# waldstein94/Stratified-Transformer

Measured on AMD Instinct MI355X. Metric: points/sec through StratifiedAttention fwd+bwd, 100k-pt scene, higher is better.
Workload: dtype f32

## Files before the change

include/pointops2_hip.h:

```cpp
#ifndef POINTOPS2_HIP_H
#define POINTOPS2_HIP_H

#include <stddef.h>
#include <stdint.h>

#ifdef __cplusplus
extern "C" {
#endif

void pointops2_set_stream(void *hip_stream);
void *pointops2_get_stream(void);
const char *pointops2_last_error(void);
int pointops2_abi_version(void);
void pointops2_diag_set_fps_patience(unsigned long long ticks_100mhz);


void furthestsampling_cuda_launcher(int b, int n, const float *xyz, const int *offset,
                                    const int *new_offset, float *tmp, int *idx);

void knnquery_cuda_launcher(int m, int nsample, const float *xyz, const float *new_xyz,
                            const int *offset, const int *new_offset, int *idx, float *dist2);

void grouping_forward_cuda_launcher(int m, int nsample, int c, const float *input, const int *idx, float *output);
void grouping_backward_cuda_launcher(int m, int nsample, int c, const float *grad_output, const int *idx, float *grad_input);
// ... 103 lines not shown
void segment_softmax_forward_launcher(int N, int M, int h, const float *src, const int *offsets, float *out);
void segment_softmax_backward_launcher(int N, int M, int h, const float *out, const float *grad_out,
                                       const int *offsets, float *grad_src);
void pointops2_bbox_launcher(int N, const float *xyz, float *out6);
size_t pointops2_index_workspace_bytes(int N);
void pointops2_window_partition_launcher(int N, int b, const float *xyz, const int *offset, const float *bbox6, float size,
                                         float shift, int key_bits, int *cluster, int *order, int *starts, int *n_windows,
                                         void *ws, size_t ws_bytes);
size_t pointops2_row_order_workspace_bytes(int N);
void pointops2_row_order_launcher(int N, int M, const int *offsets, const int *index1, int *order, void *ws, size_t ws_bytes);
size_t pointops2_partitions4_workspace_bytes(int N);
void pointops2_window_partitions4_launcher(int N, int b, const float *xyz, const int *offset, const float *bbox6, float window,
                                           int *cluster, int *order, int *starts, int *n_windows, int *overflow, void *ws,
                                           size_t ws_bytes);
void pointops2_window_coord_launcher(int N, const float *xyz, const float *bbox6, float window, int shifted, float *wc);
void pointops2_sampled_buckets_launcher(int N, int m, const int *sample_idx, const int *l_order, const int *l_starts,
                                        const int *l_n_windows, int *sampled, int *ls, int *ls_starts, void *ws, size_t ws_bytes);
void pointops2_pairs_count_launcher(int N, const int *s_cluster, const int *s_starts, const int *l_cluster, const int *ls,
                                    const int *ls_starts, const float *wc, int *offsets, void *ws, size_t ws_bytes);
void pointops2_pairs_fill_launcher(int N, const float *xyz, float window, float quant, const int *s_cluster, const int *s_order,
                                   const int *s_starts, const int *l_cluster, const int *ls, const int *ls_starts, const float *wc,
                                   const int *offsets, int *index_0, int *index_1, int *rel_idx);

void csr_expand_launcher(int N, int M, const int *offsets, int *index0);

void pointops2_csr_matches_launcher(int N, int M, const int *offsets, const void *index, int index_is_int64, int *bad);

void window_logits_softmax_forward_launcher(int N, int M, int h, int hdim, const float *q, const int *index_q_offsets,
                                             const float *k, const int *index_k, const float *table_q,
                                             const float *table_k, const int *rel_idx, float *attn);
// ... 215 lines not shown
```

stratified_transformer_amd/_lib.py:

```python
import ctypes
import os
import subprocess

import torch

_HERE = os.path.dirname(os.path.abspath(__file__))
LIB_PATH = os.path.join(_HERE, "lib", "libpointops2_hip.so")
CSRC = os.path.join(_HERE, "csrc")
_lib = None

I, U, P, Z, F, D = ctypes.c_int, ctypes.c_uint, ctypes.c_void_p, ctypes.c_size_t, ctypes.c_float, ctypes.c_double
Q = ctypes.c_longlong


class LaunchOpts(ctypes.Structure):
    _fields_ = [("table_rows", I), ("key_rows", I), ("csc_offsets", P), ("csc_pair", P), ("csc_query", P), ("row_order", P),
                ("row_order_rows", I), ("workspace", P), ("workspace_bytes", Z), ("point_count", I), ("batch_count", I),
                ("fps_prev_idx", P), ("fps_prev_new_offset", P), ("fps_unordered", I)]


def with_table_rows(opts, L):
    opts = opts if opts is not None else LaunchOpts()
    opts.table_rows = int(L)
    return opts
# ... 31 lines not shown
    "subtraction_forward_cuda_launcher": [I, I, I, P, P, P, P],
    "subtraction_backward_cuda_launcher": [I, I, I, P, P, P, P],
    "aggregation_forward_cuda_launcher": [I, I, I, I, P, P, P, P, P],
    "aggregation_backward_cuda_launcher": [I, I, I, I, P, P, P, P, P, P, P, P],
    "segment_softmax_forward_launcher": [I, I, I, P, P, P],
    "window_logits_softmax_forward_launcher": [I, I, I, I, P, P, P, P, P, P, P, P],
    "window_attention_backward_launcher": [I, I, I, I] + [P] * 18,
    "segment_softmax_backward_launcher": [I, I, I, P, P, P, P],
    "csr_expand_launcher": [I, I, P, P],
    "pointops2_csr_matches_launcher": [I, I, P, P, I, P],
    "pointops2_bbox_launcher": [I, P, P],
    "pointops2_window_partition_launcher": [I, I, P, P, P, F, F, I, P, P, P, P, P, Z],
    "pointops2_window_partitions4_launcher": [I, I, P, P, P, F, P, P, P, P, P, P, Z],
    "pointops2_row_order_launcher": [I, I, P, P, P, P, Z],
    "pointops2_window_coord_launcher": [I, P, P, F, I, P],
    "pointops2_sampled_buckets_launcher": [I, I, P, P, P, P, P, P, P, P, Z],
    "pointops2_pairs_count_launcher": [I, P, P, P, P, P, P, P, P, Z],
    "pointops2_pairs_fill_launcher": [I, P, F, F, P, P, P, P, P, P, P, P, P, P, P],
    "pointops2_voxel_keys_launcher": [I, I, P, ctypes.c_double, P],
    "pointops2_crop_dist_launcher": [I, I, P, I, P],
    "pointops2_cell_plan_count_launcher": [I, I, P, P, P, P, P, P, P, P, P, P, P, P, P, P, Z],
    "pointops2_cell_plan_prepare_launcher": [I, I, P, P, P, P, P, P, Z],
    "pointops2_cell_plan_sizes_launcher": [I, P, P, P, P, P, P, P, P, P, P, P, P, P, Z],
    "pointops2_cell_plan_fill_launcher": [I, P, F, F, I, P, P, P, P, P, P, P, P, P, P, P, P],
    "pointops2_swin_quant_launcher": [I, P, P, F, F, I, P],
    "pointops2_swin_pairs_rel_launcher": [I, I, P, P, P, I, P],
    "pointops2_swin_cell_fill_launcher": [I, I, I] + [P] * 13,
    "cell_attention_forward_launcher": [P, I, I, I] + [P] * 9,
    "cell_attention_backward_launcher": [P, I, I, I] + [P] * 16,
    "cell_attention_forward_bf16_launcher": [P, I, I, I] + [P] * 9,
# ... 33 lines not shown
    "pointops2_augment_pass_launcher": [I] * 6 + [P] * 10,
    "pointops2_augment_blur_launcher": [Q, I, I, P, P, P],
    "optim_adamw_step_launcher": [I, I, P, P, Z, P, P, I],
    "optim_step_launcher": [I, I, I, P, P, Z, P, P, I, D, P],
}
RESULTS = {
    "pointops2_get_stream": ([], P),
    "pointops2_last_error": ([], ctypes.c_char_p),
    "pointops2_abi_version": ([], I),
    "pointops2_csc_workspace_bytes": ([I, I], Z),
    "pointops2_fps_workspace_bytes": ([I, I], Z),
    "pointops2_knn_workspace_bytes": ([I, I, I], Z),
    "pointops2_index_workspace_bytes": ([I], Z),
    "pointops2_partitions4_workspace_bytes": ([I], Z),
    "pointops2_row_order_workspace_bytes": ([I], Z),
    "pointops2_cell_plan_workspace_bytes": ([I], Z),
    "pointops2_cell_forward_variant": ([P, I, I, I, I], I),
    "pointops2_evaltile_max_parts": ([], I),
    "pointops2_optim_workspace_bytes": ([I, I], Z),
    "pointops2_optim_step_workspace_bytes": ([I, I, Q], Z),
}
OPTIM_KINDS = {"adamw": 0, "sgd": 1}

CELL_FWD = {"error": -1, "none": 0, "mfma64": 1, "mfma80": 2, "valu80": 3, "valu160": 4}
ROW_TYPES = {torch.float32: 0, torch.float16: 1, torch.bfloat16: 2}
ACTIVATIONS = {"none": 0, "relu": 1, "leaky_relu": 2, "tanh": 3}


def cell_forward_variant(plan, h, L, bf16=False, hdim=16):
    arg = None if plan is None else plan.c_arg() if hasattr(plan, "c_arg") else ctypes.byref(plan)
# ... 72 lines not shown
```

stratified_transformer_amd/csrc/fps_bucket.hip:

```cpp
#include "fps_common.h"
#include <hipcub/hipcub.hpp>
#include <cstdlib>

namespace p2 {

constexpr int FPS_MAX_BUCKETS = 2048;

__device__ __forceinline__ unsigned row0_max_u32(unsigned v) {
    v = dpp_step<0xB1, 0xF>(v);
    v = dpp_step<0x4E, 0xF>(v);
    v = dpp_step<0x141, 0xF>(v);
    v = dpp_step<0x140, 0xF>(v);
    return (unsigned)__builtin_amdgcn_readfirstlane((int)v);
}
__device__ __forceinline__ unsigned long long wmax64(unsigned long long v) {
    const unsigned hi = (unsigned)(v >> 32), lo = (unsigned)v;
    const unsigned mh = wave_max_u32(hi);
    const unsigned ml = wave_max_u32(hi == mh ? lo : 0u);
    return ((unsigned long long)mh << 32) | ml;
}

constexpr int BBOX_T = 1024;
__global__ __launch_bounds__(BBOX_T) void fps_bbox_kernel(const float *__restrict__ xyz, const int *__restrict__ offset,
                                                          float *__restrict__ bbox) {
// ... 569 lines not shown
        hipLaunchKernelGGL((fps_bucket_kernel<NBL, FPS_NW, true>), dim3(b), dim3(FPS_NW * 64), 0, st, Bref, log2B, BSZ, xyz, offset, new_offset, pts,
                           rank, prev_idx, prev_offset, verified, idx);
    else
        hipLaunchKernelGGL((fps_bucket_kernel<NBL, FPS_NW, false>), dim3(b), dim3(FPS_NW * 64), 0, st, Bref, log2B, BSZ, xyz, offset, new_offset, pts,
                           rank, prev_idx, prev_offset, verified, idx);
}

static size_t al(size_t x) { return (x + 255) & ~(size_t)255; }
static int bits_for(int b) {
    int r = 1;
    while ((1 << r) < b) r++;
    return r;
}
constexpr int FPS_HEAD = 256;

static size_t fps_cub_bytes(int b, int N) {
    size_t bytes = 0;
    (void)hipcub::DeviceRadixSort::SortPairs(nullptr, bytes, (const unsigned long long *)nullptr, (unsigned long long *)nullptr,
                                             (const int *)nullptr, (int *)nullptr, N, 0, 32 + bits_for(b), (hipStream_t) nullptr);
    return bytes;
}

__global__ void fps_head_offsets_kernel(int b, int head, const int *__restrict__ new_offset, int *__restrict__ head_offset) {
    if (threadIdx.x != 0 || blockIdx.x != 0) return;
    int acc = 0;
    for (int i = 0; i < b; i++) {
        const int m = new_offset[i] - (i ? new_offset[i - 1] : 0);
        acc += min(m, head);
        head_offset[i] = acc;
    }
}

bool fps_bucket_launch(const Launch &ln, int b, int n, int Bref, int log2B, const float *xyz, const int *offset,
                       const int *new_offset, int *idx) {
    const pointops2_launch_opts &o = ln.opts;
    const int N_total = o.point_count;
// ... 9 lines not shown
    int *vals_in = (int *)p; p += f4;
    unsigned long long *keys_in = (unsigned long long *)p; p += f8;
    unsigned long long *keys_out = (unsigned long long *)p; p += f8;
    float *bbox = (float *)p; p += al((size_t)b * 6 * 4);
    int *inv = (int *)p; p += f4;
    unsigned long long *thr = (unsigned long long *)p; p += f8;
    int *first_bad = (int *)p; p += al((size_t)b * 4);
    void *xchg = p; p += al((size_t)b * LZ_XCHG);
    int *head_offset = (int *)p; p += al((size_t)b * 4);
    int *head_idx = (int *)p; p += al((size_t)b * FPS_HEAD * 4);
    void *cub_tmp = p;
    size_t cub_bytes = o.workspace_bytes - (size_t)(p - reinterpret_cast<char *>(o.workspace));
    if (o.fps_prev_idx == nullptr) {
        hipLaunchKernelGGL(fps_bbox_kernel, dim3(b), dim3(BBOX_T), 0, st, xyz, offset, bbox);
        hipLaunchKernelGGL(fps_morton_kernel, dim3(div_up(N_total, 256)), dim3(256), 0, st, N_total, b, xyz, offset, bbox, keys_in, vals_in);
        hipError_t e = hipcub::DeviceRadixSort::SortPairs(cub_tmp, cub_bytes, keys_in, keys_out, (const int *)vals_in, sorig, N_total, 0,
                                                          32 + bits_for(b), st);
        if (e != hipSuccess) { set_error(hipGetErrorString(e)); return true; }
        hipLaunchKernelGGL(fps_gather_kernel, dim3(div_up(N_total, 256)), dim3(256), 0, st, N_total, b, Bref, log2B, xyz, offset, sorig, pts, rank, inv);
    }
    const int *verified = nullptr;
    if (!o.fps_unordered) {
        hipLaunchKernelGGL(fps_verify_init_kernel, dim3(div_up(b, 64)), dim3(64), 0, st, b, offset, new_offset, first_bad);
        hipLaunchKernelGGL(fps_verify_threshold_kernel, dim3(1, b), dim3(VER_T), 0, st, Bref, log2B, 1, xyz, offset, new_offset, first_bad, thr);
        hipLaunchKernelGGL(fps_verify_scan_kernel, dim3(div_up(n, VER_P), b), dim3(VER_T), 0, st, Bref, log2B, 1, 64, xyz, offset, new_offset, thr, first_bad);
        hipLaunchKernelGGL(fps_verify_threshold_kernel, dim3(div_up(n, VER_P), b), dim3(VER_T), 0, st, Bref, log2B, 64, xyz, offset, new_offset, first_bad, thr);
        hipLaunchKernelGGL(fps_verify_scan_kernel, dim3(div_up(n, VER_P), b), dim3(VER_T), 0, st, Bref, log2B, 64, 0x7fffffff, xyz, offset, new_offset, thr, first_bad);
        hipLaunchKernelGGL(fps_rebuild_kernel, dim3(div_up(n, VER_P), b), dim3(VER_T), 0, st, xyz, offset, o.fps_prev_new_offset, first_bad, inv, pts);
        verified = first_bad;
    }
    const int BSZ = 64 * div_up(n, 64 * FPS_MAX_BUCKETS);
    const int nbuckets = div_up(n, BSZ);
// ... 37 lines not shown
```

stratified_transformer_amd/csrc/index.hip:

```cpp
#include "common.h"
#include <hipcub/hipcub.hpp>

namespace p2 {

__device__ __forceinline__ float div_floor(float a, float b) {
    if (b == 0.f) return __fdiv_rn(a, b);
    const float mod = fmodf(a, b);
    float div = __fdiv_rn(__fsub_rn(a, mod), b);
    if ((mod != 0.f) && ((b < 0.f) != (mod < 0.f))) div = __fsub_rn(div, 1.f);
    float floordiv;
    if (div != 0.f) {
        floordiv = floorf(div);
        if (__fsub_rn(div, floordiv) > 0.5f) floordiv = __fadd_rn(floordiv, 1.f);
    } else {
        floordiv = copysignf(0.f, __fdiv_rn(a, b));
    }
    return floordiv;
}

__global__ __launch_bounds__(1024) void bbox_kernel(int N, const float *__restrict__ xyz, float *__restrict__ out6) {
    __shared__ float red[6][16];
    const int tid = threadIdx.x;
    float mn[3] = {INFINITY, INFINITY, INFINITY}, mx[3] = {-INFINITY, -INFINITY, -INFINITY};
    for (int i0 = tid; i0 < N; i0 += 4 * 1024) {
// ... 352 lines not shown
        unsigned w = (jl >= nd && !coord_differs(wc, i, j)) ? 0x80000000u : 0u;
#pragma unroll
        for (int a = 0; a < 3; a++) {
            const int b = min(max(qi[a] - q[(size_t)j * 3 + a] + bias, 0), L - 1);
            w |= (unsigned)b << (8 * a);
        }
        row[jl] = w;
        if (il == 0) {
            cell_keys[kb + jl] = j;
            kcell[kb + jl] = cid;
        }
    }
}

static size_t al(size_t x) { return (x + 255) & ~(size_t)255; }
static size_t sort64_bytes(int N) {
    size_t bytes = 0;
    (void)hipcub::DeviceRadixSort::SortPairs(nullptr, bytes, (const unsigned long long *)nullptr, (unsigned long long *)nullptr,
                                             (const int *)nullptr, (int *)nullptr, N, 0, 64, (hipStream_t) nullptr);
    return bytes;
}
static size_t sort32_bytes(int N) {
    size_t bytes = 0;
    (void)hipcub::DeviceRadixSort::SortPairs(nullptr, bytes, (const unsigned *)nullptr, (unsigned *)nullptr, (const int *)nullptr, (int *)nullptr, N, 0, 32,
                                             (hipStream_t) nullptr);
    return bytes;
}
__global__ void row_order_key_kernel(int N, int M, const int *__restrict__ offs, const int *__restrict__ idx1, unsigned *__restrict__ keys,
                                     int *__restrict__ vals) {
    const int i = blockIdx.x * blockDim.x + threadIdx.x;
    if (i >= N) return;
    const int s = offs[i], e = offs[i + 1];
    keys[i] = (s >= 0 && s < e && s < M) ? (unsigned)idx1[s] : 0xffffffffu;
    vals[i] = i;
}
static size_t scan_bytes(int N) {
    size_t bytes = 0;
    (void)hipcub::DeviceScan::InclusiveSum(nullptr, bytes, (const int *)nullptr, (int *)nullptr, N, (hipStream_t) nullptr);
    size_t b2 = 0;
    (void)hipcub::DeviceScan::ExclusiveSum(nullptr, b2, (const int *)nullptr, (int *)nullptr, N, (hipStream_t) nullptr);
    return bytes > b2 ? bytes : b2;
}
// ... 21 lines not shown
                                         size_t ws_bytes) {
    const hipStream_t st = begin_launch().stream;
    if (N <= 0) return;
    if (ws_bytes < pointops2_index_workspace_bytes(N)) { set_error("pointops2_window_partition: workspace too small"); return; }
    char *p = reinterpret_cast<char *>(ws);
    unsigned long long *keys_in = (unsigned long long *)p; p += al((size_t)N * 8);
    unsigned long long *keys_out = (unsigned long long *)p; p += al((size_t)N * 8);
    int *vals_in = (int *)p; p += al(((size_t)N + 1) * 4);
    int *flags = (int *)p; p += al(((size_t)N + 1) * 4);
    int *rank = (int *)p; p += al(((size_t)N + 1) * 4);
    p += al(((size_t)N + 1) * 4);
    void *tmp = p;
    size_t tmp_bytes = ws_bytes - (size_t)(p - reinterpret_cast<char *>(ws));
    const int g = div_up(N, 256);
    hipLaunchKernelGGL(voxel_key_kernel, dim3(g), dim3(256), 0, st, N, b, xyz, offset, bbox6, size, shift, keys_in, vals_in);
    hipError_t e = hipcub::DeviceRadixSort::SortPairs(tmp, tmp_bytes, (const unsigned long long *)keys_in, keys_out, (const int *)vals_in, order, N,
                                                      0, (key_bits > 0 && key_bits < 64) ? key_bits : 64, st);
    if (e != hipSuccess) { set_error(hipGetErrorString(e)); return; }
    hipLaunchKernelGGL(boundary_flag_kernel, dim3(g), dim3(256), 0, st, N, keys_out, flags);
    e = hipcub::DeviceScan::InclusiveSum(tmp, tmp_bytes, (const int *)flags, rank, N, st);
    if (e != hipSuccess) { set_error(hipGetErrorString(e)); return; }
    hipLaunchKernelGGL(partition_finish_kernel, dim3(g), dim3(256), 0, st, N, order, flags, rank, cluster, starts, n_windows);
    check_launch();
}

size_t pointops2_row_order_workspace_bytes(int N) {
    if (N <= 0) return 0;
    return 2 * al((size_t)N * 4) + al((size_t)N * 4) + al(sort32_bytes(N));
}

void pointops2_row_order_launcher(int N, int M, const int *offsets, const int *index1, int *order, void *ws, size_t ws_bytes) {
    const hipStream_t st = begin_launch().stream;
    if (N <= 0) return;
    if (ws_bytes < pointops2_row_order_workspace_bytes(N)) { set_error("pointops2_row_order: workspace too small"); return; }
    char *p = reinterpret_cast<char *>(ws);
    unsigned *keys_in = (unsigned *)p; p += al((size_t)N * 4);
    unsigned *keys_out = (unsigned *)p; p += al((size_t)N * 4);
    int *vals_in = (int *)p; p += al((size_t)N * 4);
    size_t tmp_bytes = ws_bytes - (size_t)(p - reinterpret_cast<char *>(ws));
    hipLaunchKernelGGL(row_order_key_kernel, dim3(div_up(N, 256)), dim3(256), 0, st, N, M, offsets, index1, keys_in, vals_in);
    hipError_t e = hipcub::DeviceRadixSort::SortPairs(p, tmp_bytes, (const unsigned *)keys_in, keys_out, (const int *)vals_in, order, N, 0, 32, st);
    if (e != hipSuccess) { set_error(hipGetErrorString(e)); return; }
    check_launch();
}

size_t pointops2_partitions4_workspace_bytes(int N) {
    if (N <= 0) return 0;
    const size_t n4 = 4 * (size_t)N;
    return 2 * al(n4 * 8) + 3 * al((n4 + 1) * 4) + al(sort64_bytes((int)n4)) + al(scan_bytes((int)n4 + 1));
}

void pointops2_window_partitions4_launcher(int N, int b, const float *xyz, const int *offset, const float *bbox6, float window, int *cluster,
                                           int *order, int *starts, int *n_windows, int *overflow, void *ws, size_t ws_bytes) {
    const hipStream_t st = begin_launch().stream;
    if (N <= 0) return;
    if ((size_t)N * 4 >= (size_t)1 << 30) { set_error("pointops2_window_partitions4: too many points"); return; }
    if (ws_bytes < pointops2_partitions4_workspace_bytes(N)) { set_error("pointops2_window_partitions4: workspace too small"); return; }
    const int n4 = 4 * N;
    char *p = reinterpret_cast<char *>(ws);
    unsigned long long *keys_in = (unsigned long long *)p; p += al((size_t)n4 * 8);
    unsigned long long *keys_out = (unsigned long long *)p; p += al((size_t)n4 * 8);
    int *vals_in = (int *)p; p += al(((size_t)n4 + 1) * 4);
    int *flags = (int *)p; p += al(((size_t)n4 + 1) * 4);
    int *rank = (int *)p; p += al(((size_t)n4 + 1) * 4);
    void *tmp = p;
    size_t tmp_bytes = ws_bytes - (size_t)(p - reinterpret_cast<char *>(ws));
    int batch_bits = 0;
    while ((1 << batch_bits) < b) batch_bits++;
    const int g = div_up(n4, 256);
    (void)hipMemsetAsync(overflow, 0, sizeof(int), st);
    hipLaunchKernelGGL(voxel_key4_kernel, dim3(g), dim3(256), 0, st, N, b, xyz, offset, bbox6, window, batch_bits, keys_in, vals_in, overflow);
    hipError_t e = hipcub::DeviceRadixSort::SortPairs(tmp, tmp_bytes, (const unsigned long long *)keys_in, keys_out, (const int *)vals_in, order, n4,
                                                      0, 32 + batch_bits, st);
    if (e != hipSuccess) { set_error(hipGetErrorString(e)); return; }
    hipLaunchKernelGGL(boundary_flag_kernel, dim3(g), dim3(256), 0, st, n4, keys_out, flags);
    e = hipcub::DeviceScan::InclusiveSum(tmp, tmp_bytes, (const int *)flags, rank, n4, st);
    if (e != hipSuccess) { set_error(hipGetErrorString(e)); return; }
    hipLaunchKernelGGL(partition_finish4_kernel, dim3(g), dim3(256), 0, st, N, order, flags, rank, cluster, starts, n_windows);
    check_launch();
}

void pointops2_window_coord_launcher(int N, const float *xyz, const float *bbox6, float window, int shifted, float *wc) {
    const hipStream_t st = begin_launch().stream;
    if (N <= 0) return;
    hipLaunchKernelGGL(window_coord_kernel, dim3(div_up(N * 3, 256)), dim3(256), 0, st, N, xyz, bbox6, window, shifted, wc);
    check_launch();
}

// ... 72 lines not shown
    w.tmp_bytes = ws_bytes - (size_t)(p - reinterpret_cast<char *>(ws));
    return w;
}

void pointops2_cell_plan_prepare_launcher(int N, int max_queries, const int *s_cluster, const int *l_cluster, int *cell_order,
                                          int *parent_first, int *counts, void *ws, size_t ws_bytes) {
    const hipStream_t st = begin_launch().stream;
    if (N <= 0) return;
    if (ws_bytes < pointops2_cell_plan_workspace_bytes(N)) { set_error("pointops2_cell_plan_prepare: workspace too small"); return; }
    CellWs w = cell_ws(N, ws, ws_bytes);
    const int g = div_up(N, 256);
    int lbits = 1;
    while ((1ll << lbits) <= (long long)N) lbits++;
    (void)hipMemsetAsync(counts, 0, 8 * sizeof(int), st);
    hipLaunchKernelGGL(cell_key_kernel, dim3(g), dim3(256), 0, st, N, lbits, s_cluster, l_cluster, w.keys_in, w.vals_in);
    hipError_t e = hipcub::DeviceRadixSort::SortPairs(w.tmp, w.tmp_bytes, (const unsigned long long *)w.keys_in, w.keys_out,
                                                      (const int *)w.vals_in, cell_order, N, 0, 2 * lbits, st);
    if (e != hipSuccess) { set_error(hipGetErrorString(e)); return; }
    hipLaunchKernelGGL(boundary_flag_kernel, dim3(g), dim3(256), 0, st, N, w.keys_out, w.flags);
    e = hipcub::DeviceScan::InclusiveSum(w.tmp, w.tmp_bytes, (const int *)w.flags, w.rank, N, st);
    if (e != hipSuccess) { set_error(hipGetErrorString(e)); return; }
    int *prank = w.tile_of, *srank = reinterpret_cast<int *>(w.work_key);
    hipLaunchKernelGGL(cell_run_start_kernel, dim3(g), dim3(256), 0, st, N, w.flags, w.rank, w.nk_of);
    (void)hipMemcpyAsync(prank, w.rank, (size_t)N * sizeof(int), hipMemcpyDeviceToDevice, st);
    if (max_queries > 0) {
        hipLaunchKernelGGL(cell_split_flag_kernel, dim3(g), dim3(256), 0, st, N, max_queries, w.rank, w.nk_of, w.flags);
        e = hipcub::DeviceScan::InclusiveSum(w.tmp, w.tmp_bytes, (const int *)w.flags, w.rank, N, st);
        if (e != hipSuccess) { set_error(hipGetErrorString(e)); return; }
    }
    (void)hipMemcpyAsync(srank, w.rank, (size_t)N * sizeof(int), hipMemcpyDeviceToDevice, st);
    hipLaunchKernelGGL(cell_parent_kernel, dim3(g), dim3(256), 0, st, N, w.flags, srank, prank, w.nk_of, parent_first, counts);
    check_launch();
// ... 2 lines not shown
void pointops2_cell_plan_sizes_launcher(int N, const int *s_cluster, const int *s_starts, const int *l_cluster, const int *ls_starts,
                                        const int *cell_order, int *qcell, int *cell_desc, int *cell_qstart, int *cell_kbase,
                                        int *cell_pbase, int *cell_perm, int *counts, void *ws, size_t ws_bytes) {
    const hipStream_t st = begin_launch().stream;
    if (N <= 0) return;
    if (ws_bytes < pointops2_cell_plan_workspace_bytes(N)) { set_error("pointops2_cell_plan_sizes: workspace too small"); return; }
    CellWs w = cell_ws(N, ws, ws_bytes);
    const int g = div_up(N, 256);
    hipLaunchKernelGGL(cell_describe_kernel, dim3(g), dim3(256), 0, st, N, cell_order, w.flags, w.rank, s_cluster, s_starts, l_cluster, ls_starts,
                       qcell, cell_qstart, cell_desc, w.nk_of, counts);
    hipLaunchKernelGGL(cell_tile_kernel, dim3(div_up(N + 1, 256)), dim3(256), 0, st, N, counts, cell_qstart, w.nk_of, w.tile_of, w.work_key, w.vals_in);
    hipError_t e = hipcub::DeviceScan::ExclusiveSum(w.tmp, w.tmp_bytes, (const int *)w.nk_of, cell_kbase, N + 1, st);
    if (e != hipSuccess) { set_error(hipGetErrorString(e)); return; }
    e = hipcub::DeviceScan::ExclusiveSum(w.tmp, w.tmp_bytes, (const int *)w.tile_of, cell_pbase, N + 1, st);
    if (e != hipSuccess) { set_error(hipGetErrorString(e)); return; }
    e = hipcub::DeviceRadixSort::SortPairs(w.tmp, w.tmp_bytes, (const unsigned *)w.work_key, (unsigned *)w.keys_out, (const int *)w.vals_in,
                                           cell_perm, N, 0, 32, st);
    if (e != hipSuccess) { set_error(hipGetErrorString(e)); return; }
    hipLaunchKernelGGL(cell_totals_kernel, dim3(1), dim3(64), 0, st, N, cell_kbase, cell_pbase, counts);
    check_launch();
}

void pointops2_cell_plan_count_launcher(int N, int max_queries, const int *s_cluster, const int *s_starts, const int *l_cluster,
                                        const int *ls_starts, int *cell_order, int *qcell, int *cell_desc, int *cell_qstart,
                                        int *cell_kbase, int *cell_pbase, int *cell_perm, int *parent_first, int *counts, void *ws,
                                        size_t ws_bytes) {
    pointops2_cell_plan_prepare_launcher(N, max_queries, s_cluster, l_cluster, cell_order, parent_first, counts, ws, ws_bytes);
    if (state().error != nullptr) return;
    pointops2_cell_plan_sizes_launcher(N, s_cluster, s_starts, l_cluster, ls_starts, cell_order, qcell, cell_desc, cell_qstart, cell_kbase,
                                       cell_pbase, cell_perm, counts, ws, ws_bytes);
}

// ... 51 lines not shown
```

stratified_transformer_amd/csrc/knn_grid.hip:

```cpp
#include "common.h"
#include <hipcub/hipcub.hpp>

namespace p2 {

constexpr int KNN_CELL_CAP = 1 << 18;

struct KnnPlan {
    float lo[3];
    float c, inv_c;
    int dims[3];
    int ncell;
};

__global__ void knn_plan_kernel(int b, int n, const float *__restrict__ bbox, KnnPlan *plan) {
    if (threadIdx.x || blockIdx.x) return;
    float lo[3] = {INFINITY, INFINITY, INFINITY}, hi[3] = {-INFINITY, -INFINITY, -INFINITY};
    for (int i = 0; i < b; i++)
        for (int a = 0; a < 3; a++) {
            lo[a] = fminf(lo[a], bbox[i * 6 + a]);
            hi[a] = fmaxf(hi[a], bbox[i * 6 + 3 + a]);
        }
    float ext[3];
    double vol = 1.0;
    for (int a = 0; a < 3; a++) {
// ... 320 lines not shown
        }
        for (int i = 0; i < k; i++) {
            idx[(size_t)pt * k + i] = hi[i * BS + tid];
            dist2[(size_t)pt * k + i] = hd[i * BS + tid];
        }
    }
}

static size_t al(size_t x) { return (x + 255) & ~(size_t)255; }
static int bits_for_cells(int b) {
    long long tot = (long long)KNN_CELL_CAP * b;
    int r = 1;
    while ((1ll << r) < tot) r++;
    return r;
}
static size_t knn_cub_bytes(int n, int b) {
    size_t bytes = 0;
    (void)hipcub::DeviceRadixSort::SortPairs(nullptr, bytes, (const unsigned *)nullptr, (unsigned *)nullptr, (const int *)nullptr,
                                             (int *)nullptr, n, 0, bits_for_cells(b), (hipStream_t) nullptr);
    return bytes;
}
static size_t knn_ws_bytes(int n, int m, int b) {
    return al(sizeof(KnnPlan)) + al((size_t)b * 24) + 4 * al((size_t)n * 4) + al((size_t)n * 16) +
           al(((size_t)KNN_CELL_CAP * b + 1) * 4) + al((size_t)m * 4) + al(256) + 4 * al((size_t)m * 4) +
           al(knn_cub_bytes(max(n, m), b));
}

bool knn_grid_launch(const Launch &ln, int m, int k, const float *xyz, const float *new_xyz, const int *offset,
                     const int *new_offset, int *idx, float *dist2) {
    const pointops2_launch_opts &o = ln.opts;
    const int n = o.point_count, b = o.batch_count;
    if (o.workspace == nullptr || n <= 0 || b <= 0 || (long long)KNN_CELL_CAP * b > (1ll << 30)) return false;
    if (o.workspace_bytes < knn_ws_bytes(n, m, b)) return false;
    if ((long long)m * n < (1ll << 22)) return false;
    const hipStream_t st = ln.stream;
    char *p = reinterpret_cast<char *>(o.workspace);
// ... 6 lines not shown
    float4 *rec = (float4 *)p; p += al((size_t)n * 16);
    int *cell_start = (int *)p; p += al(((size_t)KNN_CELL_CAP * b + 1) * 4);
    int *replay = (int *)p; p += al((size_t)m * 4);
    int *replay_count = (int *)p; p += al(256);
    unsigned *qkeys_in = (unsigned *)p; p += al((size_t)m * 4);
    unsigned *qkeys_out = (unsigned *)p; p += al((size_t)m * 4);
    int *qvals_in = (int *)p; p += al((size_t)m * 4);
    int *qperm = (int *)p; p += al((size_t)m * 4);
    void *cub_tmp = p;
    size_t cub_bytes = o.workspace_bytes - (size_t)(p - reinterpret_cast<char *>(o.workspace));

    (void)hipMemsetAsync(replay_count, 0, sizeof(int), st);
    launch_bbox(b, xyz, offset, bbox, st);
    hipLaunchKernelGGL(knn_plan_kernel, dim3(1), dim3(1), 0, st, b, n, bbox, plan);
    hipLaunchKernelGGL(knn_cell_kernel, dim3(div_up(n, 256)), dim3(256), 0, st, n, b, xyz, offset, plan, keys_in, vals_in);
    hipError_t e = hipcub::DeviceRadixSort::SortPairs(cub_tmp, cub_bytes, (const unsigned *)keys_in, keys_out, (const int *)vals_in, vals_out,
                                                      n, 0, bits_for_cells(b), st);
    if (e != hipSuccess) { set_error(hipGetErrorString(e)); return true; }
    hipLaunchKernelGGL(knn_finish_kernel, dim3(div_up(n, 256)), dim3(256), 0, st, n, b, keys_out, vals_out, xyz, plan, cell_start, rec);
    hipLaunchKernelGGL(knn_cell_kernel, dim3(div_up(m, 256)), dim3(256), 0, st, m, b, new_xyz, new_offset, plan, qkeys_in, qvals_in);
    e = hipcub::DeviceRadixSort::SortPairs(cub_tmp, cub_bytes, (const unsigned *)qkeys_in, qkeys_out, (const int *)qvals_in, qperm, m, 0,
                                           bits_for_cells(b), st);
    if (e != hipSuccess) { set_error(hipGetErrorString(e)); return true; }
    if (k + 1 <= 64) {
#define P2_KNN_LANES(LQ_)                                                                                                              \
    hipLaunchKernelGGL(knn_lanes_kernel<LQ_>, dim3((unsigned)div_up64((int64_t)m * LQ_, 256)), dim3(256), 0, st, m, k, new_xyz, offset, new_offset, \
                       plan, cell_start, rec, idx, dist2, replay, replay_count, qperm)
        if (k + 1 <= 16) P2_KNN_LANES(16);
        else if (k + 1 <= 32) P2_KNN_LANES(32);
        else P2_KNN_LANES(64);
#undef P2_KNN_LANES
    } else {
        constexpr int BS = 64;
        const size_t lds = (size_t)(k + 1) * BS * 8;
        hipLaunchKernelGGL(knn_grid_kernel<BS>, dim3(div_up(m, BS)), dim3(BS), lds, st, m, k, new_xyz, offset, new_offset, plan, cell_start, rec,
                           idx, dist2, replay, replay_count, qperm);
    }
// ... 18 lines not shown
```

Measured before the change: 9.150 million.

## Replace hipcub radix sorts with custom short tiled LSD radix sort

```diff
diff --git a/include/pointops2_hip.h b/include/pointops2_hip.h
--- a/include/pointops2_hip.h
+++ b/include/pointops2_hip.h
@@ -141,6 +141,9 @@
                                            int *cluster, int *order, int *starts, int *n_windows, int *overflow, void *ws,
                                            size_t ws_bytes);
 void pointops2_window_coord_launcher(int N, const float *xyz, const float *bbox6, float window, int shifted, float *wc);
+size_t pointops2_short_sort_scratch_bytes(int n, int key_bytes);
+void pointops2_short_sort_pairs_launcher(int n, int key_bytes, int bits, const void *keys_in, void *keys_out, const int *vals_in,
+                                         int *vals_out, void *scratch, size_t scratch_bytes);
 void pointops2_sampled_buckets_launcher(int N, int m, const int *sample_idx, const int *l_order, const int *l_starts,
                                         const int *l_n_windows, int *sampled, int *ls, int *ls_starts, void *ws, size_t ws_bytes);
 void pointops2_pairs_count_launcher(int N, const int *s_cluster, const int *s_starts, const int *l_cluster, const int *ls,
diff --git a/stratified_transformer_amd/_lib.py b/stratified_transformer_amd/_lib.py
--- a/stratified_transformer_amd/_lib.py
+++ b/stratified_transformer_amd/_lib.py
@@ -69,6 +69,7 @@
     "pointops2_window_partitions4_launcher": [I, I, P, P, P, F, P, P, P, P, P, P, Z],
     "pointops2_row_order_launcher": [I, I, P, P, P, P, Z],
     "pointops2_window_coord_launcher": [I, P, P, F, I, P],
+    "pointops2_short_sort_pairs_launcher": [I, I, I, P, P, P, P, P, Z],
     "pointops2_sampled_buckets_launcher": [I, I, P, P, P, P, P, P, P, P, Z],
     "pointops2_pairs_count_launcher": [I, P, P, P, P, P, P, P, P, Z],
     "pointops2_pairs_fill_launcher": [I, P, F, F, P, P, P, P, P, P, P, P, P, P, P],
@@ -132,6 +133,7 @@
     "pointops2_index_workspace_bytes": ([I], Z),
     "pointops2_partitions4_workspace_bytes": ([I], Z),
     "pointops2_row_order_workspace_bytes": ([I], Z),
+    "pointops2_short_sort_scratch_bytes": ([I, I], Z),
     "pointops2_cell_plan_workspace_bytes": ([I], Z),
     "pointops2_cell_forward_variant": ([P, I, I, I, I], I),
     "pointops2_evaltile_max_parts": ([], I),
diff --git a/stratified_transformer_amd/csrc/fps_bucket.hip b/stratified_transformer_amd/csrc/fps_bucket.hip
--- a/stratified_transformer_amd/csrc/fps_bucket.hip
+++ b/stratified_transformer_amd/csrc/fps_bucket.hip
@@ -1,5 +1,5 @@
 #include "fps_common.h"
-#include <hipcub/hipcub.hpp>
+#include "short_sort.h"
 #include <cstdlib>
 
 namespace p2 {
@@ -607,12 +607,7 @@
 }
 constexpr int FPS_HEAD = 256;
 
-static size_t fps_cub_bytes(int b, int N) {
-    size_t bytes = 0;
-    (void)hipcub::DeviceRadixSort::SortPairs(nullptr, bytes, (const unsigned long long *)nullptr, (unsigned long long *)nullptr,
-                                             (const int *)nullptr, (int *)nullptr, N, 0, 32 + bits_for(b), (hipStream_t) nullptr);
-    return bytes;
-}
+static size_t fps_cub_bytes(int b, int N) { return short_sort_scratch_bytes(N, 8); }
 
 __global__ void fps_head_offsets_kernel(int b, int head, const int *__restrict__ new_offset, int *__restrict__ head_offset) {
     if (threadIdx.x != 0 || blockIdx.x != 0) return;
@@ -652,8 +647,8 @@
     if (o.fps_prev_idx == nullptr) {
         hipLaunchKernelGGL(fps_bbox_kernel, dim3(b), dim3(BBOX_T), 0, st, xyz, offset, bbox);
         hipLaunchKernelGGL(fps_morton_kernel, dim3(div_up(N_total, 256)), dim3(256), 0, st, N_total, b, xyz, offset, bbox, keys_in, vals_in);
-        hipError_t e = hipcub::DeviceRadixSort::SortPairs(cub_tmp, cub_bytes, keys_in, keys_out, (const int *)vals_in, sorig, N_total, 0,
-                                                          32 + bits_for(b), st);
+        hipError_t e = short_sort_pairs(st, (const unsigned long long *)keys_in, keys_out, (const int *)vals_in, sorig, N_total, 32 + bits_for(b),
+                                        cub_tmp, cub_bytes);
         if (e != hipSuccess) { set_error(hipGetErrorString(e)); return true; }
         hipLaunchKernelGGL(fps_gather_kernel, dim3(div_up(N_total, 256)), dim3(256), 0, st, N_total, b, Bref, log2B, xyz, offset, sorig, pts, rank, inv);
     }
diff --git a/stratified_transformer_amd/csrc/index.hip b/stratified_transformer_amd/csrc/index.hip
--- a/stratified_transformer_amd/csrc/index.hip
+++ b/stratified_transformer_amd/csrc/index.hip
@@ -1,4 +1,5 @@
 #include "common.h"
+#include "short_sort.h"
 #include <hipcub/hipcub.hpp>
 
 namespace p2 {
@@ -390,18 +391,8 @@
 }
 
 static size_t al(size_t x) { return (x + 255) & ~(size_t)255; }
-static size_t sort64_bytes(int N) {
-    size_t bytes = 0;
-    (void)hipcub::DeviceRadixSort::SortPairs(nullptr, bytes, (const unsigned long long *)nullptr, (unsigned long long *)nullptr,
-                                             (const int *)nullptr, (int *)nullptr, N, 0, 64, (hipStream_t) nullptr);
-    return bytes;
-}
-static size_t sort32_bytes(int N) {
-    size_t bytes = 0;
-    (void)hipcub::DeviceRadixSort::SortPairs(nullptr, bytes, (const unsigned *)nullptr, (unsigned *)nullptr, (const int *)nullptr, (int *)nullptr, N, 0, 32,
-                                             (hipStream_t) nullptr);
-    return bytes;
-}
+static size_t sort64_bytes(int N) { return short_sort_scratch_bytes(N, 8); }
+static size_t sort32_bytes(int N) { return short_sort_scratch_bytes(N, 4); }
 __global__ void row_order_key_kernel(int N, int M, const int *__restrict__ offs, const int *__restrict__ idx1, unsigned *__restrict__ keys,
                                      int *__restrict__ vals) {
     const int i = blockIdx.x * blockDim.x + threadIdx.x;
@@ -453,8 +444,8 @@
     size_t tmp_bytes = ws_bytes - (size_t)(p - reinterpret_cast<char *>(ws));
     const int g = div_up(N, 256);
     hipLaunchKernelGGL(voxel_key_kernel, dim3(g), dim3(256), 0, st, N, b, xyz, offset, bbox6, size, shift, keys_in, vals_in);
-    hipError_t e = hipcub::DeviceRadixSort::SortPairs(tmp, tmp_bytes, (const unsigned long long *)keys_in, keys_out, (const int *)vals_in, order, N,
-                                                      0, (key_bits > 0 && key_bits < 64) ? key_bits : 64, st);
+    hipError_t e = short_sort_pairs(st, (const unsigned long long *)keys_in, keys_out, (const int *)vals_in, order, N,
+                                    (key_bits > 0 && key_bits < 64) ? key_bits : 64, tmp, tmp_bytes);
     if (e != hipSuccess) { set_error(hipGetErrorString(e)); return; }
     hipLaunchKernelGGL(boundary_flag_kernel, dim3(g), dim3(256), 0, st, N, keys_out, flags);
     e = hipcub::DeviceScan::InclusiveSum(tmp, tmp_bytes, (const int *)flags, rank, N, st);
@@ -478,7 +469,7 @@
     int *vals_in = (int *)p; p += al((size_t)N * 4);
     size_t tmp_bytes = ws_bytes - (size_t)(p - reinterpret_cast<char *>(ws));
     hipLaunchKernelGGL(row_order_key_kernel, dim3(div_up(N, 256)), dim3(256), 0, st, N, M, offsets, index1, keys_in, vals_in);
-    hipError_t e = hipcub::DeviceRadixSort::SortPairs(p, tmp_bytes, (const unsigned *)keys_in, keys_out, (const int *)vals_in, order, N, 0, 32, st);
+    hipError_t e = short_sort_pairs(st, (const unsigned *)keys_in, keys_out, (const int *)vals_in, order, N, 32, p, tmp_bytes);
     if (e != hipSuccess) { set_error(hipGetErrorString(e)); return; }
     check_launch();
 }
@@ -509,8 +500,8 @@
     const int g = div_up(n4, 256);
     (void)hipMemsetAsync(overflow, 0, sizeof(int), st);
     hipLaunchKernelGGL(voxel_key4_kernel, dim3(g), dim3(256), 0, st, N, b, xyz, offset, bbox6, window, batch_bits, keys_in, vals_in, overflow);
-    hipError_t e = hipcub::DeviceRadixSort::SortPairs(tmp, tmp_bytes, (const unsigned long long *)keys_in, keys_out, (const int *)vals_in, order, n4,
-                                                      0, 32 + batch_bits, st);
+    hipError_t e = short_sort_pairs(st, (const unsigned long long *)keys_in, keys_out, (const int *)vals_in, order, n4, 32 + batch_bits, tmp,
+                                    tmp_bytes);
     if (e != hipSuccess) { set_error(hipGetErrorString(e)); return; }
     hipLaunchKernelGGL(boundary_flag_kernel, dim3(g), dim3(256), 0, st, n4, keys_out, flags);
     e = hipcub::DeviceScan::InclusiveSum(tmp, tmp_bytes, (const int *)flags, rank, n4, st);
@@ -613,8 +604,8 @@
     while ((1ll << lbits) <= (long long)N) lbits++;
     (void)hipMemsetAsync(counts, 0, 8 * sizeof(int), st);
     hipLaunchKernelGGL(cell_key_kernel, dim3(g), dim3(256), 0, st, N, lbits, s_cluster, l_cluster, w.keys_in, w.vals_in);
-    hipError_t e = hipcub::DeviceRadixSort::SortPairs(w.tmp, w.tmp_bytes, (const unsigned long long *)w.keys_in, w.keys_out,
-                                                      (const int *)w.vals_in, cell_order, N, 0, 2 * lbits, st);
+    hipError_t e = short_sort_pairs(st, (const unsigned long long *)w.keys_in, w.keys_out, (const int *)w.vals_in, cell_order, N, 2 * lbits, w.tmp,
+                                    w.tmp_bytes);
     if (e != hipSuccess) { set_error(hipGetErrorString(e)); return; }
     hipLaunchKernelGGL(boundary_flag_kernel, dim3(g), dim3(256), 0, st, N, w.keys_out, w.flags);
     e = hipcub::DeviceScan::InclusiveSum(w.tmp, w.tmp_bytes, (const int *)w.flags, w.rank, N, st);
@@ -647,8 +638,7 @@
     if (e != hipSuccess) { set_error(hipGetErrorString(e)); return; }
     e = hipcub::DeviceScan::ExclusiveSum(w.tmp, w.tmp_bytes, (const int *)w.tile_of, cell_pbase, N + 1, st);
     if (e != hipSuccess) { set_error(hipGetErrorString(e)); return; }
-    e = hipcub::DeviceRadixSort::SortPairs(w.tmp, w.tmp_bytes, (const unsigned *)w.work_key, (unsigned *)w.keys_out, (const int *)w.vals_in,
-                                           cell_perm, N, 0, 32, st);
+    e = short_sort_pairs(st, (const unsigned *)w.work_key, (unsigned *)w.keys_out, (const int *)w.vals_in, cell_perm, N, 32, w.tmp, w.tmp_bytes);
     if (e != hipSuccess) { set_error(hipGetErrorString(e)); return; }
     hipLaunchKernelGGL(cell_totals_kernel, dim3(1), dim3(64), 0, st, N, cell_kbase, cell_pbase, counts);
     check_launch();
diff --git a/stratified_transformer_amd/csrc/knn_grid.hip b/stratified_transformer_amd/csrc/knn_grid.hip
--- a/stratified_transformer_amd/csrc/knn_grid.hip
+++ b/stratified_transformer_amd/csrc/knn_grid.hip
@@ -1,5 +1,5 @@
 #include "common.h"
-#include <hipcub/hipcub.hpp>
+#include "short_sort.h"
 
 namespace p2 {
 
@@ -358,12 +358,7 @@
     while ((1ll << r) < tot) r++;
     return r;
 }
-static size_t knn_cub_bytes(int n, int b) {
-    size_t bytes = 0;
-    (void)hipcub::DeviceRadixSort::SortPairs(nullptr, bytes, (const unsigned *)nullptr, (unsigned *)nullptr, (const int *)nullptr,
-                                             (int *)nullptr, n, 0, bits_for_cells(b), (hipStream_t) nullptr);
-    return bytes;
-}
+static size_t knn_cub_bytes(int n, int b) { return short_sort_scratch_bytes(n, 4); }
 static size_t knn_ws_bytes(int n, int m, int b) {
     return al(sizeof(KnnPlan)) + al((size_t)b * 24) + 4 * al((size_t)n * 4) + al((size_t)n * 16) +
            al(((size_t)KNN_CELL_CAP * b + 1) * 4) + al((size_t)m * 4) + al(256) + 4 * al((size_t)m * 4) +
@@ -400,13 +395,11 @@
     launch_bbox(b, xyz, offset, bbox, st);
     hipLaunchKernelGGL(knn_plan_kernel, dim3(1), dim3(1), 0, st, b, n, bbox, plan);
     hipLaunchKernelGGL(knn_cell_kernel, dim3(div_up(n, 256)), dim3(256), 0, st, n, b, xyz, offset, plan, keys_in, vals_in);
-    hipError_t e = hipcub::DeviceRadixSort::SortPairs(cub_tmp, cub_bytes, (const unsigned *)keys_in, keys_out, (const int *)vals_in, vals_out,
-                                                      n, 0, bits_for_cells(b), st);
+    hipError_t e = short_sort_pairs(st, (const unsigned *)keys_in, keys_out, (const int *)vals_in, vals_out, n, bits_for_cells(b), cub_tmp, cub_bytes);
     if (e != hipSuccess) { set_error(hipGetErrorString(e)); return true; }
     hipLaunchKernelGGL(knn_finish_kernel, dim3(div_up(n, 256)), dim3(256), 0, st, n, b, keys_out, vals_out, xyz, plan, cell_start, rec);
     hipLaunchKernelGGL(knn_cell_kernel, dim3(div_up(m, 256)), dim3(256), 0, st, m, b, new_xyz, new_offset, plan, qkeys_in, qvals_in);
-    e = hipcub::DeviceRadixSort::SortPairs(cub_tmp, cub_bytes, (const unsigned *)qkeys_in, qkeys_out, (const int *)qvals_in, qperm, m, 0,
-                                           bits_for_cells(b), st);
+    e = short_sort_pairs(st, (const unsigned *)qkeys_in, qkeys_out, (const int *)qvals_in, qperm, m, bits_for_cells(b), cub_tmp, cub_bytes);
     if (e != hipSuccess) { set_error(hipGetErrorString(e)); return true; }
     if (k + 1 <= 64) {
 #define P2_KNN_LANES(LQ_)                                                                                                              \
diff --git a/stratified_transformer_amd/csrc/short_sort.h b/stratified_transformer_amd/csrc/short_sort.h
--- /dev/null
+++ b/stratified_transformer_amd/csrc/short_sort.h
@@ -0,0 +1,18 @@
+#pragma once
+#include <hip/hip_runtime.h>
+#include <stddef.h>
+
+namespace p2 {
+
+constexpr int SHORT_SORT_DIGIT_BITS = 8;
+constexpr int SHORT_SORT_TILE = 4096;
+constexpr int SHORT_SORT_MAX_N = 1 << 20;
+
+size_t short_sort_scratch_bytes(int n, int key_bytes);
+
+hipError_t short_sort_pairs(hipStream_t st, const unsigned *keys_in, unsigned *keys_out, const int *vals_in, int *vals_out, int n, int bits,
+                            void *scratch, size_t scratch_bytes);
+hipError_t short_sort_pairs(hipStream_t st, const unsigned long long *keys_in, unsigned long long *keys_out, const int *vals_in, int *vals_out,
+                            int n, int bits, void *scratch, size_t scratch_bytes);
+
+}
diff --git a/stratified_transformer_amd/csrc/short_sort.hip b/stratified_transformer_amd/csrc/short_sort.hip
--- /dev/null
+++ b/stratified_transformer_amd/csrc/short_sort.hip
@@ -0,0 +1,272 @@
+#include "common.h"
+#include "short_sort.h"
+#include <hipcub/hipcub.hpp>
+
+namespace p2 {
+
+namespace {
+
+constexpr int SS_RADIX = 1 << SHORT_SORT_DIGIT_BITS;
+constexpr int SS_THREADS = 1024, SS_WAVES = SS_THREADS / 64, SS_ROUNDS = SHORT_SORT_TILE / SS_THREADS;
+static_assert(SS_RADIX == 256 && SS_THREADS == 4 * SS_RADIX, "the table sums and the scan below are written for 256 digits and 1024 threads");
+static_assert(SS_ROUNDS * SS_THREADS == SHORT_SORT_TILE && SHORT_SORT_MAX_N / SHORT_SORT_TILE <= 256, "tile geometry");
+
+size_t al(size_t x) { return (x + 255) & ~(size_t)255; }
+
+__device__ __forceinline__ unsigned long long digit_peers(unsigned digit, bool valid) {
+    unsigned long long peers = __ballot(valid);
+#pragma unroll
+    for (int b = 0; b < SHORT_SORT_DIGIT_BITS; b++) {
+        const bool bit = (digit >> b) & 1u;
+        const unsigned long long with = __ballot(valid && bit);
+        peers &= bit ? with : ~with;
+    }
+    return valid ? peers : 0ull;
+}
+
+template <typename K>
+struct Items {
+    K key[SS_ROUNDS];
+    int val[SS_ROUNDS];
+    int digit[SS_ROUNDS];
+    int rank[SS_ROUNDS];
+};
+
+template <typename K>
+__device__ __forceinline__ void rank_tile(const K *keys, const int *vals, int n, int tile_base, int shift, unsigned mask,
+                                          int *wcount, Items<K> &it) {
+    const int wave = threadIdx.x >> 6, lane = threadIdx.x & 63;
+    int *mine = wcount + wave * SS_RADIX;
+#pragma unroll
+    for (int r = 0; r < SS_ROUNDS; r++) {
+        const int i = tile_base + wave * (64 * SS_ROUNDS) + r * 64 + lane;
+        const bool valid = i < n;
+        it.key[r] = valid ? keys[i] : (K)0;
+        it.val[r] = valid ? vals[i] : 0;
+        const unsigned d = (unsigned)(it.key[r] >> shift) & mask;
+        const unsigned long long peers = digit_peers(d, valid);
+        const int leader = valid ? __ffsll((long long)peers) - 1 : lane;
+        int before = 0;
+        if (valid && lane == leader) {
+            before = mine[d];
+            mine[d] = before + __popcll(peers);
+        }
+        before = __shfl(before, leader, 64);
+        it.digit[r] = valid ? (int)d : -1;
+        it.rank[r] = before + __popcll(peers & ((1ull << lane) - 1ull));
+    }
+}
+
+__device__ __forceinline__ void exclusive_scan_radix(int *s) {
+    const int l = threadIdx.x;
+    const int a0 = s[4 * l], a1 = s[4 * l + 1], a2 = s[4 * l + 2], a3 = s[4 * l + 3];
+    const int sum = a0 + a1 + a2 + a3;
+    int inc = sum;
+#pragma unroll
+    for (int o = 1; o < 64; o <<= 1) {
+        const int t = __shfl_up(inc, o, 64);
+        if (l >= o) inc += t;
+    }
+    const int ex = inc - sum;
+    s[4 * l] = ex;
+    s[4 * l + 1] = ex + a0;
+    s[4 * l + 2] = ex + a0 + a1;
+    s[4 * l + 3] = ex + a0 + a1 + a2;
+}
+
+__device__ __forceinline__ void prefix_waves(int *wcount, int d, int first) {
+#pragma unroll
+    for (int w = 0; w < SS_WAVES; w++) {
+        const int c = wcount[w * SS_RADIX + d];
+        wcount[w * SS_RADIX + d] = first;
+        first += c;
+    }
+}
+
+template <typename K>
+__device__ __forceinline__ void write_tile(const Items<K> &it, const int *wcount, K *keys_out, int *vals_out) {
+    const int *mine = wcount + (threadIdx.x >> 6) * SS_RADIX;
+#pragma unroll
+    for (int r = 0; r < SS_ROUNDS; r++) {
+        if (it.digit[r] < 0) continue;
+        const int pos = mine[it.digit[r]] + it.rank[r];
+        keys_out[pos] = it.key[r];
+        vals_out[pos] = it.val[r];
+    }
+}
+
+template <typename K>
+__global__ __launch_bounds__(SS_THREADS) void short_sort_count_kernel(const K *__restrict__ keys, int n, int shift, unsigned mask,
+                                                                      int *__restrict__ counts) {
+    __shared__ int hist[SS_RADIX];
+    if (threadIdx.x < SS_RADIX) hist[threadIdx.x] = 0;
+    __syncthreads();
+    const int lane = threadIdx.x & 63;
+#pragma unroll
+    for (int r = 0; r < SS_ROUNDS; r++) {
+        const int i = blockIdx.x * SHORT_SORT_TILE + r * SS_THREADS + threadIdx.x;
+        const bool valid = i < n;
+        const unsigned d = valid ? (unsigned)(keys[i] >> shift) & mask : 0u;
+        const unsigned long long peers = digit_peers(d, valid);
+        if (valid && lane == __ffsll((long long)peers) - 1) atomicAdd(&hist[d], __popcll(peers));
+    }
+    __syncthreads();
+    if (threadIdx.x < SS_RADIX) counts[blockIdx.x * SS_RADIX + threadIdx.x] = hist[threadIdx.x];
+}
+
+template <typename K>
+__global__ __launch_bounds__(SS_THREADS) void short_sort_scatter_kernel(const K *__restrict__ keys_in, const int *__restrict__ vals_in,
+                                                                        K *__restrict__ keys_out, int *__restrict__ vals_out, int n, int shift,
+                                                                        unsigned mask, const int *__restrict__ counts) {
+    __shared__ int wcount[SS_WAVES * SS_RADIX];
+    __shared__ int part_total[4 * SS_RADIX], part_before[4 * SS_RADIX];
+    __shared__ int total[SS_RADIX], before[SS_RADIX];
+    const int tile = blockIdx.x, tiles = gridDim.x;
+    for (int j = threadIdx.x; j < SS_WAVES * SS_RADIX; j += SS_THREADS) wcount[j] = 0;
+    {
+        const int d = threadIdx.x & (SS_RADIX - 1), q = threadIdx.x >> SHORT_SORT_DIGIT_BITS;
+        int all = 0, low = 0;
+        for (int t = q; t < tiles; t += 4) {
+            const int c = counts[t * SS_RADIX + d];
+            all += c;
+            if (t < tile) low += c;
+        }
+        part_total[threadIdx.x] = all;
+        part_before[threadIdx.x] = low;
+    }
+    __syncthreads();
+    if (threadIdx.x < SS_RADIX) {
+        const int d = threadIdx.x;
+        total[d] = part_total[d] + part_total[SS_RADIX + d] + part_total[2 * SS_RADIX + d] + part_total[3 * SS_RADIX + d];
+        before[d] = part_before[d] + part_before[SS_RADIX + d] + part_before[2 * SS_RADIX + d] + part_before[3 * SS_RADIX + d];
+    }
+    Items<K> it;
+    rank_tile(keys_in, vals_in, n, tile * SHORT_SORT_TILE, shift, mask, wcount, it);
+    __syncthreads();
+    if (threadIdx.x < 64) exclusive_scan_radix(total);
+    __syncthreads();
+    if (threadIdx.x < SS_RADIX) prefix_waves(wcount, threadIdx.x, total[threadIdx.x] + before[threadIdx.x]);
+    __syncthreads();
+    write_tile(it, wcount, keys_out, vals_out);
+}
+
+template <typename K>
+__global__ __launch_bounds__(SS_THREADS) void short_sort_tile_kernel(const K *__restrict__ keys_in, const int *__restrict__ vals_in, K *keys_out,
+                                                                     int *vals_out, K *keys_alt, int *vals_alt, int n, int bits, int passes) {
+    __shared__ int wcount[SS_WAVES * SS_RADIX];
+    __shared__ int total[SS_RADIX];
+    const K *ksrc = keys_in;
+    const int *vsrc = vals_in;
+    for (int p = 0; p < passes; p++) {
+        const int shift = p * SHORT_SORT_DIGIT_BITS, left = bits - shift;
+        const unsigned mask = left >= SHORT_SORT_DIGIT_BITS ? SS_RADIX - 1 : left > 0 ? (1u << left) - 1u : 0u;
+        const bool to_out = ((passes - 1 - p) & 1) == 0;
+        K *kdst = to_out ? keys_out : keys_alt;
+        int *vdst = to_out ? vals_out : vals_alt;
+        for (int j = threadIdx.x; j < SS_WAVES * SS_RADIX; j += SS_THREADS) wcount[j] = 0;
+        __syncthreads();
+        Items<K> it;
+        rank_tile(ksrc, vsrc, n, 0, shift, mask, wcount, it);
+        __syncthreads();
+        if (threadIdx.x < SS_RADIX) {
+            int s = 0;
+#pragma unroll
+            for (int w = 0; w < SS_WAVES; w++) s += wcount[w * SS_RADIX + threadIdx.x];
+            total[threadIdx.x] = s;
+        }
+        __syncthreads();
+        if (threadIdx.x < 64) exclusive_scan_radix(total);
+        __syncthreads();
+        if (threadIdx.x < SS_RADIX) prefix_waves(wcount, threadIdx.x, total[threadIdx.x]);
+        __syncthreads();
+        write_tile(it, wcount, kdst, vdst);
+        __syncthreads();
+        ksrc = kdst;
+        vsrc = vdst;
+    }
+}
+
+template <typename K>
+hipError_t sort_pairs(hipStream_t st, const K *keys_in, K *keys_out, const int *vals_in, int *vals_out, int n, int bits, void *scratch,
+                      size_t scratch_bytes) {
+    if (n <= 0) return hipSuccess;
+    bits = bits < 0 ? 0 : bits > (int)sizeof(K) * 8 ? (int)sizeof(K) * 8 : bits;
+    if (scratch == nullptr || scratch_bytes < short_sort_scratch_bytes(n, (int)sizeof(K))) return hipErrorInvalidValue;
+    if (n > SHORT_SORT_MAX_N) return hipcub::DeviceRadixSort::SortPairs(scratch, scratch_bytes, keys_in, keys_out, vals_in, vals_out, n, 0, bits, st);
+    const int tiles = div_up(n, SHORT_SORT_TILE), passes = bits > 0 ? div_up(bits, SHORT_SORT_DIGIT_BITS) : 1;
+    char *p = reinterpret_cast<char *>(scratch);
+    int *counts = (int *)p; p += al((size_t)tiles * SS_RADIX * sizeof(int));
+    K *keys_alt = (K *)p; p += al((size_t)n * sizeof(K));
+    int *vals_alt = (int *)p;
+    if (tiles == 1) {
+        hipLaunchKernelGGL(short_sort_tile_kernel<K>, dim3(1), dim3(SS_THREADS), 0, st, keys_in, vals_in, keys_out, vals_out, keys_alt, vals_alt, n, bits,
+                           passes);
+        return hipGetLastError();
+    }
+    const K *ksrc = keys_in;
+    const int *vsrc = vals_in;
+    for (int ps = 0; ps < passes; ps++) {
+        const int shift = ps * SHORT_SORT_DIGIT_BITS, left = bits - shift;
+        const unsigned mask = left >= SHORT_SORT_DIGIT_BITS ? SS_RADIX - 1 : left > 0 ? (1u << left) - 1u : 0u;
+        const bool to_out = ((passes - 1 - ps) & 1) == 0;
+        K *kdst = to_out ? keys_out : keys_alt;
+        int *vdst = to_out ? vals_out : vals_alt;
+        hipLaunchKernelGGL(short_sort_count_kernel<K>, dim3(tiles), dim3(SS_THREADS), 0, st, ksrc, n, shift, mask, counts);
+        hipLaunchKernelGGL(short_sort_scatter_kernel<K>, dim3(tiles), dim3(SS_THREADS), 0, st, ksrc, vsrc, kdst, vdst, n, shift, mask,
+                           (const int *)counts);
+        ksrc = kdst;
+        vsrc = vdst;
+    }
+    return hipGetLastError();
+}
+
+}
+
+size_t short_sort_scratch_bytes(int n, int key_bytes) {
+    if (n <= 0) return 0;
+    if (n > SHORT_SORT_MAX_N) {
+        size_t bytes = 0;
+        if (key_bytes == 8)
+            (void)hipcub::DeviceRadixSort::SortPairs(nullptr, bytes, (const unsigned long long *)nullptr, (unsigned long long *)nullptr,
+                                                     (const int *)nullptr, (int *)nullptr, n, 0, 64, (hipStream_t) nullptr);
+        else
+            (void)hipcub::DeviceRadixSort::SortPairs(nullptr, bytes, (const unsigned *)nullptr, (unsigned *)nullptr, (const int *)nullptr,
+                                                     (int *)nullptr, n, 0, 32, (hipStream_t) nullptr);
+        return bytes;
+    }
+    return al((size_t)div_up(n, SHORT_SORT_TILE) * SS_RADIX * sizeof(int)) + al((size_t)n * (size_t)key_bytes) + al((size_t)n * sizeof(int));
+}
+
+hipError_t short_sort_pairs(hipStream_t st, const unsigned *keys_in, unsigned *keys_out, const int *vals_in, int *vals_out, int n, int bits,
+                            void *scratch, size_t scratch_bytes) {
+    return sort_pairs(st, keys_in, keys_out, vals_in, vals_out, n, bits, scratch, scratch_bytes);
+}
+hipError_t short_sort_pairs(hipStream_t st, const unsigned long long *keys_in, unsigned long long *keys_out, const int *vals_in, int *vals_out,
+                            int n, int bits, void *scratch, size_t scratch_bytes) {
+    return sort_pairs(st, keys_in, keys_out, vals_in, vals_out, n, bits, scratch, scratch_bytes);
+}
+
+}
+
+using namespace p2;
+
+extern "C" {
+
+size_t pointops2_short_sort_scratch_bytes(int n, int key_bytes) {
+    if (key_bytes != 4 && key_bytes != 8) return 0;
+    return short_sort_scratch_bytes(n, key_bytes);
+}
+
+void pointops2_short_sort_pairs_launcher(int n, int key_bytes, int bits, const void *keys_in, void *keys_out, const int *vals_in, int *vals_out,
+                                         void *scratch, size_t scratch_bytes) {
+    const hipStream_t st = begin_launch().stream;
+    if (key_bytes != 4 && key_bytes != 8) { set_error("pointops2_short_sort_pairs: key_bytes must be 4 or 8"); return; }
+    if (n <= 0) return;
+    const hipError_t e = key_bytes == 8 ? short_sort_pairs(st, (const unsigned long long *)keys_in, (unsigned long long *)keys_out, vals_in, vals_out,
+                                                           n, bits, scratch, scratch_bytes)
+                                        : short_sort_pairs(st, (const unsigned *)keys_in, (unsigned *)keys_out, vals_in, vals_out, n, bits, scratch,
+                                                           scratch_bytes);
+    if (e != hipSuccess) set_error(hipGetErrorString(e));
+}
+
+}
```

Result: slower. 8.861 million (-3.2%).
